# alexmillerdb/two_tower_recommender_model

Hardware: AMD Instinct MI355X
Metric: training pairs/sec at batch 8192 (per GPU) (higher is better)
Workload: dtype fp32; 1 GPU; northstar: 100M items x 50M users, emb_dim 128, towers [128, 64], single-hot uniform ids; global_batch=8192, per_gpu_batch=8192, emb_dim=128, tower_dtype=bf16 (MFMA, fp32 acc), parallelism=single-gpu hipgraph

## Files before the change

### two_tower_recommender_model_amd/csrc/tower.hip

```cpp
#include <vector>

#include "tt_common.h"
#include "dedup.h"
#include "shard.h"

namespace tt {

typedef __attribute__((ext_vector_type(8))) __bf16 bf16x8;
typedef __attribute__((ext_vector_type(4))) float f32x4;
typedef __attribute__((ext_vector_type(4))) __bf16 bf16x4;

constexpr int TR = 32;
constexpr int MAXW = 128;
constexpr int XCH = 128;
constexpr int LSTR = MAXW + 8;
constexpr int FSTR = MAXW + 4;
constexpr int MAXL = 4;

__device__ __forceinline__ int64_t strip_at(int64_t f, int64_t m, int64_t nf) {
  return (((m >> 5) * nf + f) << 5) + (m & 31);
}

struct TowerArgs {
  tt_tower_shape_t s;
// ... 1411 lines not shown
  } else {
#pragma unroll
    for (int mt = 0; mt < MTI; ++mt) {
      const int c = 8 * (mt >> 1) + 2 * q + (mt & 1);
      const f32x4 v = *reinterpret_cast<const f32x4*>(xw + n * IN + 4 * (c ^ n));
      xv[mt] = r >= 0 ? v : (f32x4)(0.f);
    }
#pragma unroll
    for (int s2 = 0; s2 < NI; ++s2) xb[s2] = rk_pack(xv[2 * s2], xv[2 * s2 + 1]);
  }
  uint32_t word = 0u;
  float s_old = 0.f;
  if (UPD) {
    if (blockIdx.x == 0 && threadIdx.x == 0) {
      const int32_t nh = a.dd.ctr[0];
      a.dd.ctr[2] = nh;
      a.dd.ctr[0] = 0;
    }
    word = reinterpret_cast<const uint32_t*>(&a.dd.slots[cl >= 0 ? cl : 0].word)[0];
    s_old = (t ? a.us[1] : a.us[0])[r >= 0 ? r : 0];
  }
  __builtin_amdgcn_sched_barrier(0);
  const char* img0 = wimg + t * RK_IMG_T;
  const char* img1 = img0 + RK_W0 * 256;
  f32x4 acc[8];
  if (!TDBG(512)) rk_strip<NI>(xb, a.xt + (int64_t)t * a.in_max * a.Bp + m * a.in_max, q);
  rk_gemm<8, NI, false>(acc, img0, xb, lane);
  RK_STAMP(4);
  bf16x8 hb[4];
#pragma unroll
  for (int s = 0; s < 4; ++s) {
    f32x4 u0, u1;
#pragma unroll
    for (int j = 0; j < 4; ++j) {
      u0[j] = fmaxf(acc[2 * s][j] + b0v[2 * s][j], 0.f);
      u1[j] = fmaxf(acc[2 * s + 1][j] + b0v[2 * s + 1][j], 0.f);
    }
    hb[s] = rk_pack(u0, u1);
  }
  if (!TDBG(256)) rk_strip<4>(hb, a.act + ((int64_t)t * MAXL + 0) * MAXW * a.Bp + m * MAXW, q);
  f32x4 uo[4];
  rk_gemm<4, 4, false>(acc, img1, hb, lane);
#pragma unroll
  for (int mt = 0; mt < 4; ++mt) uo[mt] = acc[mt];
#pragma unroll
  for (int mt = 0; mt < 4; ++mt) {
#pragma unroll
    for (int j = 0; j < 4; ++j) uo[mt][j] = fmaxf(uo[mt][j] + b1v[mt][j], 0.f);
    const int c = 8 * (mt >> 1) + 2 * q + (mt & 1);
    *reinterpret_cast<f32x4*>(&xo[t][h][n * 64 + ((c ^ n) << 2)]) = uo[mt];
  }
  RK_STAMP(5);
  RK_STAMP(6);
  __syncthreads();
  RK_STAMP(7);
  f32x4 vo[4];
#pragma unroll
  for (int mt = 0; mt < 4; ++mt) {
    const int c = 8 * (mt >> 1) + 2 * q + (mt & 1);
    vo[mt] = *reinterpret_cast<const f32x4*>(&xo[t ^ 1][h][n * 64 + ((c ^ n) << 2)]);
  }
  float gs[4];
#pragma unroll
  for (int mt = 0; mt < 4; ++mt) {
    float e = 0.f;
#pragma unroll
    for (int j = 0; j < 4; ++j) e = fmaf(uo[mt][j], vo[mt][j], e);
    gs[mt] = e;
  }
  float c0 = gs[0] + gs[1], c1 = gs[2] + gs[3];
  c0 += __shfl_xor(c0, 16, 64);
  c1 += __shfl_xor(c1, 16, 64);
  c0 += __shfl_xor(c0, 32, 64);
  c1 += __shfl_xor(c1, 32, 64);
  const float d = c0 + c1;
  float lo = 0.f, dl = 0.f;
  if (live) {
    const float x = d, y = rk_label(lab_raw, a.label_dtype);
    const float e = __expf(-fabsf(x));
    const float l1p = e < 1e-4f ? e * (1.f - 0.5f * e) : __logf(1.f + e);
    const float lsig = fminf(x, 0.f) - l1p;
    lo = (1.f - y) * x - lsig;
    const float rc = __builtin_amdgcn_rcpf(1.f + e);
    dl = ((x >= 0.f ? rc : e * rc) - y) * (a.grad_scale / (float)B);
  }
  if (t == 0 && q == 0) lrow[16 * h + n] = lo;
  float z1[16];
  bf16x8 z1b[4];
#pragma unroll
  for (int mt = 0; mt < 4; ++mt)
#pragma unroll
    for (int j = 0; j < 4; ++j) z1[4 * mt + j] = live && uo[mt][j] > 0.f ? dl * vo[mt][j] : 0.f;
#pragma unroll
  for (int s = 0; s < 2; ++s) {
    bf16x8 v;
#pragma unroll
    for (int j = 0; j < 8; ++j) v[j] = (__bf16)z1[8 * s + j];
    z1b[s] = v;
  }
  RK_STAMP(8);
  rk_gemm<8, 2, true>(acc, img1, z1b, lane);
  float z0[32];
  bf16x8 z0b[4];
#pragma unroll
  for (int mt = 0; mt < 8; ++mt)
#pragma unroll
    for (int j = 0; j < 4; ++j)
      z0[4 * mt + j] = live && (float)hb[mt >> 1][4 * (mt & 1) + j] > 0.f ? acc[mt][j] : 0.f;
#pragma unroll
  for (int s = 0; s < 4; ++s) {
    bf16x8 v;
#pragma unroll
    for (int j = 0; j < 8; ++j) v[j] = (__bf16)z0[8 * s + j];
    z0b[s] = v;
  }
  if (!TDBG(512)) rk_strip<2>(z1b, a.dzt + ((int64_t)t * MAXL + 1) * MAXW * a.Bp + m * MAXW, q);
  if (!TDBG(128)) rk_strip<4>(z0b, a.dzt + ((int64_t)t * MAXL + 0) * MAXW * a.Bp + m * MAXW, q);
  RK_STAMP(9);
  rk_gemm<MTI, 4, true>(acc, img0, z0b, lane);
  RK_STAMP(10);
  float* grow;
  bool store_dx;
  if (IDX) {
    const int32_t po = (int32_t)pout_raw.lo;
    store_dx = r >= 0 && po >= 0;
    grow = (t ? a.gdst[1] : a.gdst[0]) + (int64_t)(store_dx ? po : 0) * IN;
    if (a.xd.W) grow = reinterpret_cast<float*>(px_row(a.xd, store_dx ? po : 0, IN * 4));
  } else {
    grow = live ? a.gpooled + m * a.ldp + a.s.in_col[t] : nullptr;
    store_dx = live;
  }
  if (UPD) {
    float e2[2];
#pragma unroll
    for (int hh = 0; hh < 2; ++hh) {
      const float s0 = rw_sq4(acc[0 + hh]), s1 = rw_sq4(acc[2 + hh]);
      float c2;
      if constexpr (IN == 128) {
        const float s2 = rw_sq4(acc[4 + hh]), s3 = rw_sq4(acc[6 + hh]);
        c2 = (s0 + s2) + (s1 + s3);
      } else {
        c2 = s0 + s1;
      }
      c2 += __shfl_xor(c2, 32, 64);
      c2 += __shfl_xor(c2, 16, 64);
      e2[hh] = c2;
    }
    RK_STAMP2(0);
    const float sq = e2[0] + e2[1];
    const float snew = rw_state(s_old, sq, IN);
    const float step = rw_step(snew, a.ulr, a.ueps);
    const uint32_t cnt = word & (uint32_t)DD_CNT_MASK;
    const bool single = r >= 0 && cl >= 0 && cnt == 1u;
    {
      const bool mul = q == 0 && r >= 0 && cl >= 0 && cnt >= 2u && cnt <= (uint32_t)DD_INL;
      const uint64_t bal = __ballot(mul);
      const int seg = tile * 4 + wid;
      if (seg < a.dd.nseg) {
        if (mul) a.dd.multi[(int64_t)seg * DD_SEGW + 1 + __popcll(bal & ((1ull << lane) - 1))] = cl;
        if (lane == 0) a.dd.multi[(int64_t)seg * DD_SEGW] = __popcll(bal);
      }
    }
#pragma unroll
    for (int mt = 0; mt < MTI; ++mt) {
      const int c = 8 * (mt >> 1) + 2 * q + (mt & 1);
      *reinterpret_cast<f32x4*>(xw + n * IN + 4 * (c ^ n)) = rw_apply(xv[mt], acc[mt], step);
    }
    RK_STAMP2(1);
    asm volatile("" ::: "memory");
    {
      const int rr0 = lane / CPR, pc = lane % CPR;
      float* wtab = t ? a.uw[1] : a.uw[0];
#pragma unroll
      for (int i = 0; i < 16 / RPI; ++i) {
        const int row = RPI * i + rr0;
        const int64_t rid = __shfl((long long)r, row, 64);
        const int sg = __shfl((int)single, row, 64);
        const f32x4 w = *reinterpret_cast<const f32x4*>(xw + row * IN + 4 * pc);
        if (sg) *reinterpret_cast<f32x4*>(wtab + rid * IN + 4 * (pc ^ row)) = w;
      }
    }
    RK_STAMP2(2);
    if (single) {
      if (q == 0) {
        (t ? a.us[1] : a.us[0])[r] = snew;
        a.dd.slots[cl].word = DD_EMPTY;
      }
      store_dx = a.pooled_out != nullptr;
    }
  }
  if (store_dx) {
#pragma unroll
    for (int mt = 0; mt < MTI; ++mt)
      *reinterpret_cast<f32x4*>(grow + 32 * (mt >> 1) + 8 * q + 4 * (mt & 1)) = acc[mt];
  }
  RK_STAMP2(3);
  if (t == 0 && q == 0 && live) a.logits[m] = d;
  if (!IDX && !POOL && a.pooled_out && live) {
    float* prow = a.pooled_out + m * a.ldp + a.s.in_col[t];
#pragma unroll
    for (int mt = 0; mt < MTI; ++mt) *reinterpret_cast<f32x4*>(prow + 32 * (mt >> 1) + 8 * q + 4 * (mt & 1)) = xv[mt];
  }
  RK_STAMP(11);
  RK_STAMP(12);
  rk_colsum<32>(z0, n);
  rk_colsum<16>(z1, n);
  auto feat = [&](int k) { return 32 * ((k >> 2) >> 1) + 8 * q + 4 * ((k >> 2) & 1) + (k & 3); };
  if (h == 1) {
    bsum[t][feat(2 * n)] = z0[0];
    bsum[t][feat(2 * n + 1)] = z0[1];
    bsum[t][RK_W0 + feat(n)] = z1[0];
  }
  RK_STAMP(13);
  __syncthreads();
  RK_STAMP(14);
  if (h == 0) {
    float* db0 = a.dbpart + (((int64_t)t * MAXL + 0) * a.nwg + tile) * MAXW;
    float* db1 = a.dbpart + (((int64_t)t * MAXL + 1) * a.nwg + tile) * MAXW;
    db0[feat(2 * n)] = z0[0] + bsum[t][feat(2 * n)];
    db0[feat(2 * n + 1)] = z0[1] + bsum[t][feat(2 * n + 1)];
    db1[feat(n)] = z1[0] + bsum[t][RK_W0 + feat(n)];
    if (t == 0 && lane == 0) {
      float p = 0.f;
      for (int i = 0; i < TR; ++i) p += lrow[i];
      a.loss_part[tile] = p;
    }
  }
  if (!UPD && a.dd_on && q == 0) dd_insert_defer_finish_at(a.dd, pend, li, tile, 16 * wid + n);
  if constexpr (IDX) {
    if (cpd) *cpd = cpv;
    if (a.xd.W) {
      for (int64_t u = (int64_t)blockIdx.x * cp_per + threadIdx.x + 256; u < cp_end; u += 256) {
        const uint4* s2;
        uint4* d2;
        if (px_copy_unit(a.xd, u, s2, d2)) *d2 = *s2;
      }
    }
    if (a.xd.epoch && blockIdx.x == 0 && threadIdx.x == 0)
      __hip_atomic_fetch_add(a.xd.epoch, 1, __ATOMIC_RELAXED, __HIP_MEMORY_SCOPE_AGENT);
  }
  RK_STAMP(15);
}
template <bool UPD, bool IDX = false, int IN = 128, bool POOL = false>
__global__ void __launch_bounds__(RK_THREADS) tower_rows_kernel(TowerArgs a) {
  tower_rows_body<UPD, IDX, IN, POOL>(a);
}


struct WgradTile {
  int32_t t, l, n0, k0;
};


struct WgradArgs {
  const __bf16* xt;
  const __bf16* act;
  const __bf16* dzt;
  float* slab;
  int64_t P;
  int64_t B;
  int64_t in_max;
  int64_t Bp;
  int S;
  int64_t mslice;
  int ntiles;
  int64_t woff[2][MAXL];
  int64_t boff[2][MAXL];
  int32_t K[2][MAXL];
  int32_t width[MAXL];
  int L;
  const float* dbpart;
  int nwg;
  const float* loss_part;
  float* loss;
  int nbias;
  int64_t tiles_off;
  int64_t* step_state;
  float* adam_pre;
  float lr, beta1, beta2;
  int lds;
  int rm;
  int32_t t2_code[16];
#if TT_EXPERIMENTS
  int64_t* stamps;
#endif
  DedupWs dd;
  int n_res;
};

#if TT_EXPERIMENTS
#define T2_STAMP(k) \
  do { if (a.stamps && threadIdx.x == 0) a.stamps[(int64_t)blockIdx.x * 8 + (k)] = (int64_t)__builtin_amdgcn_s_memrealtime(); } while (0)
#else
#define T2_STAMP(k) do { } while (0)
#endif

constexpr int T2_NT = 64;
constexpr int T2_MB = 32;
constexpr int T2_PF = 8;
constexpr int T2_STR = T2_MB + 8;
constexpr int T2_ROWS = T2_NT + MAXW;
constexpr int T2_LDS = 2 * T2_ROWS * T2_STR * 2;
constexpr int T2_RED = 3 * 64 * 16 * 4;
constexpr int T2_SMEM0 = T2_LDS > T2_RED ? T2_LDS : T2_RED;
constexpr int T2_SMEM = T2_SMEM0 > DD_SMEM ? T2_SMEM0 : DD_SMEM;


__device__ __forceinline__ void wgrad_lds_block(const WgradArgs& a, int lb, char* smem) {
  __bf16* buf = reinterpret_cast<__bf16*>(smem);
  const int tid = threadIdx.x, lane = tid & 63, wid = tid >> 6;
  const int r = lane & 15, q = lane >> 4;
  const int s = __builtin_amdgcn_readfirstlane(lb / a.ntiles), ti = __builtin_amdgcn_readfirstlane(lb % a.ntiles);
  T2_STAMP(0);
  const int code = a.t2_code[ti];
  const int t = code & 15, l = (code >> 4) & 15, n0 = code >> 8;
  const int K = a.K[t][l];
  const int NT = min(T2_NT, a.width[l] - n0);
  const int64_t B = a.B;
  const __bf16* Z = a.dzt + ((int64_t)t * MAXL + l) * MAXW * a.Bp;
  const __bf16* A = l == 0 ? a.xt + (int64_t)t * a.in_max * a.Bp : a.act + ((int64_t)t * MAXL + l - 1) * MAXW * a.Bp;
  const int64_t anf = l == 0 ? a.in_max : MAXW;
  const int64_t mb = (int64_t)s * a.mslice;
  const int64_t me = min(mb + a.mslice, B);
  const int seg = (tid & 3) * 8, frow = tid >> 2;
  const __bf16* src[3];
  int64_t tstr[3];
#pragma unroll
  for (int i = 0; i < 3; ++i) {
    const int f = frow + 64 * i;
    src[i] = f < T2_NT ? (f < NT ? Z + ((int64_t)(n0 + f) << 5) : nullptr)
                       : (f - T2_NT < K ? A + ((int64_t)(f - T2_NT) << 5) : nullptr);
    tstr[i] = (f < T2_NT ? (int64_t)MAXW : anf) << 5;
  }
  const int nh = wid >> 1, kh = wid & 1;
  f32x4 acc[2][4];
#pragma unroll
  for (int i = 0; i < 2; ++i)
#pragma unroll
    for (int j = 0; j < 4; ++j) acc[i][j] = (f32x4)(0.f);
  for (int64_t p0 = mb; p0 < me; p0 += T2_PF * T2_MB) {
    bf16x8 ld[T2_PF][3];
#pragma unroll
    for (int c = 0; c < T2_PF; ++c) {
      const int64_t m = p0 + c * T2_MB + seg;
#pragma unroll
      for (int i = 0; i < 3; ++i)
        ld[c][i] = (src[i] && m < me) ? *reinterpret_cast<const bf16x8*>(src[i] + (m >> 5) * tstr[i] + seg)
                                      : (bf16x8)(__bf16)0.f;
    }
#pragma unroll
    for (int c = 0; c < T2_PF; ++c) {
      if (p0 + c * T2_MB >= me) break;
      __bf16* d = buf + (c & 1) * T2_ROWS * T2_STR;
#pragma unroll
      for (int i = 0; i < 3; ++i)
        if (src[i]) *reinterpret_cast<bf16x8*>(d + (frow + 64 * i) * T2_STR + seg) = ld[c][i];
      __syncthreads();
      if (c == 0 && p0 == mb) T2_STAMP(1);
      bf16x8 fa[2], fb[4];
#pragma unroll
      for (int i = 0; i < 2; ++i) fa[i] = *reinterpret_cast<const bf16x8*>(d + (nh * 32 + i * 16 + r) * T2_STR + q * 8);
#pragma unroll
      for (int j = 0; j < 4; ++j)
        fb[j] = *reinterpret_cast<const bf16x8*>(d + (T2_NT + kh * 64 + j * 16 + r) * T2_STR + q * 8);
#pragma unroll
      for (int i = 0; i < 2; ++i)
#pragma unroll
        for (int j = 0; j < 4; ++j)
          if (nh * 32 + i * 16 < NT && kh * 64 + j * 16 < K)
            acc[i][j] = __builtin_amdgcn_mfma_f32_16x16x32_bf16(fa[i], fb[j], acc[i][j], 0, 0, 0);
    }
  }
  T2_STAMP(2);
  float* dst = a.slab + (int64_t)s * a.P + a.woff[t][l];
#pragma unroll
  for (int i = 0; i < 2; ++i)
#pragma unroll
    for (int j = 0; j < 4; ++j)
      if (nh * 32 + i * 16 < NT && kh * 64 + j * 16 < K)
#pragma unroll
        for (int rr = 0; rr < 4; ++rr) {
          const int n = n0 + nh * 32 + i * 16 + q * 4 + rr;
          const int k = kh * 64 + j * 16 + r;
          dst[(int64_t)n * K + k] = acc[i][j][rr];
        }
  T2_STAMP(3);
}

constexpr int T2R_STR = 208;
static_assert(2 * TR * T2R_STR * 2 <= T2_SMEM, "the row-major staged chunks fit the tail's LDS");
__device__ __forceinline__ bf16x8 t2r_frag(const __bf16* d, int col0, int lane) {
  const int q = lane >> 4, qq = (lane >> 2) & 3, p = lane & 3;
  const __bf16* base = d + (4 * q + qq) * T2R_STR + col0 + 4 * p;
  const bf16x4 lo = __builtin_amdgcn_ds_read_tr16_b64_v4bf16((lds_bf16x4*)base);
  const bf16x4 hi = __builtin_amdgcn_ds_read_tr16_b64_v4bf16((lds_bf16x4*)(base + 16 * T2R_STR));
  return __builtin_shufflevector(lo, hi, 0, 1, 2, 3, 4, 5, 6, 7);
}
__device__ __forceinline__ void wgrad_lds_block_rm(const WgradArgs& a, int lb, char* smem) {
  __bf16* buf = reinterpret_cast<__bf16*>(smem);
  const int tid = threadIdx.x, lane = tid & 63, wid = tid >> 6;
  const int r = lane & 15, q = lane >> 4;
  const int s = __builtin_amdgcn_readfirstlane(lb / a.ntiles), ti = __builtin_amdgcn_readfirstlane(lb % a.ntiles);
  T2_STAMP(0);
  const int code = a.t2_code[ti];
  const int t = code & 15, l = (code >> 4) & 15, n0 = code >> 8;
  const int K = a.K[t][l];
  const int NT = min(T2_NT, a.width[l] - n0);
  const int64_t B = a.B;
  const __bf16* Z = a.dzt + ((int64_t)t * MAXL + l) * MAXW * a.Bp;
  const __bf16* A = l == 0 ? a.xt + (int64_t)t * a.in_max * a.Bp : a.act + ((int64_t)t * MAXL + l - 1) * MAXW * a.Bp;
  const int64_t anf = l == 0 ? a.in_max : MAXW;
  const int64_t mb = (int64_t)s * a.mslice;
  const int64_t me = min(mb + a.mslice, B);
  const char* zb = reinterpret_cast<const char*>(Z);
  const char* ab = reinterpret_cast<const char*>(A);
  const int prow0 = tid >> 3, prow1 = tid >> 4, prow2 = (tid + 256) >> 4;
  const bool ok0 = 8 * (tid & 7) < NT, ok1 = 8 * (tid & 15) < K, ok2 = 8 * ((tid + 256) & 15) < K;
  const uint32_t zstr = MAXW * 2, astr = (uint32_t)anf * 2;
  const uint32_t zo = (uint32_t)(mb + prow0) * zstr + (uint32_t)(n0 + 8 * (tid & 7)) * 2;
  const uint32_t ao1 = (uint32_t)(mb + prow1) * astr + (uint32_t)(8 * (tid & 15)) * 2;
  const uint32_t ao2 = (uint32_t)(mb + prow2) * astr + (uint32_t)(8 * ((tid + 256) & 15)) * 2;
  const int lw0 = prow0 * T2R_STR + 8 * (tid & 7);
  const int lw1 = prow1 * T2R_STR + T2_NT + 8 * (tid & 15);
  const int lw2 = prow2 * T2R_STR + T2_NT + 8 * ((tid + 256) & 15);
  const int nh = wid >> 1, kh = wid & 1;
  f32x4 acc[2][4];
#pragma unroll
  for (int i = 0; i < 2; ++i)
#pragma unroll
    for (int j = 0; j < 4; ++j) acc[i][j] = (f32x4)(0.f);
  for (int64_t p0 = mb; p0 < me; p0 += T2_PF * T2_MB) {
    bf16x8 ld[T2_PF][3];
    const uint32_t dr = (uint32_t)(p0 - mb);
    bool okc[T2_PF][3];
#pragma unroll
    for (int c = 0; c < T2_PF; ++c) {
      const uint32_t rc = dr + c * T2_MB;
      const int64_t mrow = p0 + c * T2_MB;
      okc[c][0] = ok0 && mrow + prow0 < me;
      okc[c][1] = ok1 && mrow + prow1 < me;
      okc[c][2] = ok2 && mrow + prow2 < me;
      ld[c][0] = *reinterpret_cast<const bf16x8*>(zb + zo + (okc[c][0] ? rc * zstr : 0u));
      ld[c][1] = *reinterpret_cast<const bf16x8*>(ab + ao1 + (okc[c][1] ? rc * astr : 0u));
      ld[c][2] = *reinterpret_cast<const bf16x8*>(ab + ao2 + (okc[c][2] ? rc * astr : 0u));
    }
#pragma unroll
    for (int c = 0; c < T2_PF; ++c) {
      if (p0 + c * T2_MB >= me) break;
      __bf16* d = buf + (c & 1) * TR * T2R_STR;
#pragma unroll
      for (int i = 0; i < 3; ++i)
        if (!okc[c][i]) ld[c][i] = (bf16x8)(__bf16)0.f;
      *reinterpret_cast<bf16x8*>(d + lw0) = ld[c][0];
      *reinterpret_cast<bf16x8*>(d + lw1) = ld[c][1];
      *reinterpret_cast<bf16x8*>(d + lw2) = ld[c][2];
      __syncthreads();
      if (c == 0 && p0 == mb) T2_STAMP(1);
      bf16x8 fa[2], fb[4];
#pragma unroll
      for (int i = 0; i < 2; ++i) fa[i] = t2r_frag(d, nh * 32 + i * 16, lane);
#pragma unroll
      for (int j = 0; j < 4; ++j) fb[j] = t2r_frag(d, T2_NT + kh * 64 + j * 16, lane);
#pragma unroll
      for (int i = 0; i < 2; ++i)
#pragma unroll
        for (int j = 0; j < 4; ++j)
          if (nh * 32 + i * 16 < NT && kh * 64 + j * 16 < K)
            acc[i][j] = __builtin_amdgcn_mfma_f32_16x16x32_bf16(fa[i], fb[j], acc[i][j], 0, 0, 0);
    }
  }
  T2_STAMP(2);
  float* dst = a.slab + (int64_t)s * a.P + a.woff[t][l];
#pragma unroll
  for (int i = 0; i < 2; ++i)
#pragma unroll
    for (int j = 0; j < 4; ++j)
      if (nh * 32 + i * 16 < NT && kh * 64 + j * 16 < K)
#pragma unroll
        for (int rr = 0; rr < 4; ++rr) {
          const int n = n0 + nh * 32 + i * 16 + q * 4 + rr;
          const int k = kh * 64 + j * 16 + r;
          dst[(int64_t)n * K + k] = acc[i][j][rr];
        }
  T2_STAMP(3);
}

__device__ __forceinline__ void wgrad_block(const WgradArgs& a, const WgradTile* __restrict__ tiles, int bid,
                                            char* smem) {
  float (*red)[64 * 16] = reinterpret_cast<float (*)[64 * 16]>(smem);
  const int lane = threadIdx.x & 63, wid = threadIdx.x >> 6;
  const int r = lane & 15, q = lane >> 4;
  const int64_t nwg_tiles = (int64_t)a.ntiles * a.S;
  if ((int64_t)bid >= nwg_tiles) {
    T2_STAMP(0);
    int64_t b = ((int64_t)bid - nwg_tiles) * 4 + wid;
    if (b == a.nbias) {
      b = -1;
      if (a.loss) {
        float s = 0.f;
        for (int w0 = 0; w0 < a.nwg; w0 += 512) {
          float v[8];
#pragma unroll
          for (int k = 0; k < 8; ++k) v[k] = w0 + k * 64 + lane < a.nwg ? a.loss_part[w0 + k * 64 + lane] : 0.f;
#pragma unroll
          for (int k = 0; k < 8; ++k) s += v[k];
        }
        s = wave_sum(s);
        if (lane == 0) a.loss[0] = s / (float)a.B;
      }
      if (a.adam_pre && lane == 0) {
        const int64_t t_step = a.step_state[0] + 1;
        a.step_state[0] = t_step;
        const double bc1 = 1.0 - pow((double)a.beta1, (double)t_step);
        const double bc2 = 1.0 - pow((double)a.beta2, (double)t_step);
        a.adam_pre[0] = (float)((double)a.lr / bc1);
        a.adam_pre[1] = (float)sqrt(bc2);
      }
    }
    for (int t = 0; t < 2; ++t)
      for (int l = 0; l < a.L; ++l) {
        if (b >= 0 && b < a.width[l]) {
          const float* dbp = a.dbpart + ((int64_t)t * MAXL + l) * a.nwg * MAXW + b;
          float s = 0.f;
          for (int w0 = 0; w0 < a.nwg; w0 += 512) {
            float v[8];
#pragma unroll
            for (int k = 0; k < 8; ++k) {
              const int w = w0 + k * 64 + lane;
              v[k] = w < a.nwg ? dbp[(int64_t)w * MAXW] : 0.f;
            }
#pragma unroll
            for (int k = 0; k < 8; ++k) s += v[k];
          }
          s = wave_sum(s);
          if (lane == 0) a.slab[a.boff[t][l] + b] = s;
        }
        if (b >= 0) b -= a.width[l];
      }
    T2_STAMP(3);
    return;
  }
  const int lb = xcd_remap(bid, (int)nwg_tiles);
  if (a.lds && a.rm) {
    wgrad_lds_block_rm(a, lb, smem);
    return;
  }
  if (a.lds) {
    wgrad_lds_block(a, lb, smem);
    return;
  }
  const int s = (int)(lb / a.ntiles);
  const WgradTile tl = tiles[lb % a.ntiles];
  const int64_t B = a.B;
  const __bf16* Z = a.dzt + ((int64_t)tl.t * MAXL + tl.l) * MAXW * a.Bp;
  const __bf16* A = tl.l == 0 ? a.xt + (int64_t)tl.t * a.in_max * a.Bp
                              : a.act + ((int64_t)tl.t * MAXL + tl.l - 1) * MAXW * a.Bp;
  const int64_t anf = tl.l == 0 ? a.in_max : MAXW;
  const int64_t mw = a.mslice / 4;
  int64_t mb = (int64_t)s * a.mslice + wid * mw;
  int64_t me = mb + mw;
  if (mb > B) mb = B;
  if (me > B) me = B;
  f32x4 acc[2][2];
  for (int i = 0; i < 2; ++i)
    for (int j = 0; j < 2; ++j) acc[i][j] = (f32x4)(0.f);
  const __bf16* z0 = Z + ((int64_t)(tl.n0 + r) << 5);
  const __bf16* z1 = Z + ((int64_t)(tl.n0 + 16 + r) << 5);
  const __bf16* a0 = A + ((int64_t)(tl.k0 + r) << 5);
  const __bf16* a1 = A + ((int64_t)(tl.k0 + 16 + r) << 5);
  auto zo = [&](int64_t o) { return (((o >> 5) * MAXW) << 5) + (o & 31); };
  auto ao = [&](int64_t o) { return (((o >> 5) * anf) << 5) + (o & 31); };
  int64_t m = mb;
  for (; m + 128 <= me; m += 128) {
    bf16x8 fa0[4], fa1[4], fb0[4], fb1[4];
#pragma unroll
    for (int u = 0; u < 4; ++u) {
      const int64_t o = m + 32 * u + q * 8;
      fa0[u] = *reinterpret_cast<const bf16x8*>(z0 + zo(o));
      fa1[u] = *reinterpret_cast<const bf16x8*>(z1 + zo(o));
      fb0[u] = *reinterpret_cast<const bf16x8*>(a0 + ao(o));
      fb1[u] = *reinterpret_cast<const bf16x8*>(a1 + ao(o));
    }
#pragma unroll
    for (int u = 0; u < 4; ++u) {
      acc[0][0] = __builtin_amdgcn_mfma_f32_16x16x32_bf16(fa0[u], fb0[u], acc[0][0], 0, 0, 0);
      acc[0][1] = __builtin_amdgcn_mfma_f32_16x16x32_bf16(fa0[u], fb1[u], acc[0][1], 0, 0, 0);
      acc[1][0] = __builtin_amdgcn_mfma_f32_16x16x32_bf16(fa1[u], fb0[u], acc[1][0], 0, 0, 0);
      acc[1][1] = __builtin_amdgcn_mfma_f32_16x16x32_bf16(fa1[u], fb1[u], acc[1][1], 0, 0, 0);
    }
  }
  for (; m + 32 <= me; m += 32) {
    const int64_t o = m + q * 8;
    const bf16x8 fa0 = *reinterpret_cast<const bf16x8*>(z0 + zo(o));
    const bf16x8 fa1 = *reinterpret_cast<const bf16x8*>(z1 + zo(o));
    const bf16x8 fb0 = *reinterpret_cast<const bf16x8*>(a0 + ao(o));
    const bf16x8 fb1 = *reinterpret_cast<const bf16x8*>(a1 + ao(o));
    acc[0][0] = __builtin_amdgcn_mfma_f32_16x16x32_bf16(fa0, fb0, acc[0][0], 0, 0, 0);
    acc[0][1] = __builtin_amdgcn_mfma_f32_16x16x32_bf16(fa0, fb1, acc[0][1], 0, 0, 0);
    acc[1][0] = __builtin_amdgcn_mfma_f32_16x16x32_bf16(fa1, fb0, acc[1][0], 0, 0, 0);
    acc[1][1] = __builtin_amdgcn_mfma_f32_16x16x32_bf16(fa1, fb1, acc[1][1], 0, 0, 0);
  }
  if (m < me) {
    bf16x8 fa0, fa1, fb0, fb1;
    for (int j = 0; j < 8; ++j) {
      const int64_t mm = m + q * 8 + j;
      const bool ok = mm < me;
      fa0[j] = ok ? z0[zo(mm)] : (__bf16)0.f;
      fa1[j] = ok ? z1[zo(mm)] : (__bf16)0.f;
      fb0[j] = ok ? a0[ao(mm)] : (__bf16)0.f;
      fb1[j] = ok ? a1[ao(mm)] : (__bf16)0.f;
    }
    acc[0][0] = __builtin_amdgcn_mfma_f32_16x16x32_bf16(fa0, fb0, acc[0][0], 0, 0, 0);
    acc[0][1] = __builtin_amdgcn_mfma_f32_16x16x32_bf16(fa0, fb1, acc[0][1], 0, 0, 0);
    acc[1][0] = __builtin_amdgcn_mfma_f32_16x16x32_bf16(fa1, fb0, acc[1][0], 0, 0, 0);
    acc[1][1] = __builtin_amdgcn_mfma_f32_16x16x32_bf16(fa1, fb1, acc[1][1], 0, 0, 0);
  }
  if (wid > 0) {
#pragma unroll
    for (int i = 0; i < 2; ++i)
#pragma unroll
      for (int j = 0; j < 2; ++j)
#pragma unroll
        for (int rr = 0; rr < 4; ++rr) red[wid - 1][((i * 2 + j) * 4 + rr) * 64 + lane] = acc[i][j][rr];
  }
  __syncthreads();
  if (wid > 0) return;
#pragma unroll
  for (int w = 0; w < 3; ++w)
#pragma unroll
    for (int i = 0; i < 2; ++i)
#pragma unroll
      for (int j = 0; j < 2; ++j)
#pragma unroll
        for (int rr = 0; rr < 4; ++rr) acc[i][j][rr] += red[w][((i * 2 + j) * 4 + rr) * 64 + lane];
  const int K = a.K[tl.t][tl.l];
  float* dst = a.slab + (int64_t)s * a.P + a.woff[tl.t][tl.l];
  for (int i = 0; i < 2; ++i)
    for (int j = 0; j < 2; ++j)
      for (int rr = 0; rr < 4; ++rr) {
        const int n = tl.n0 + i * 16 + q * 4 + rr;
        const int k = tl.k0 + j * 16 + r;
        dst[(int64_t)n * K + k] = acc[i][j][rr];
      }
}

__global__ void __launch_bounds__(256) tower_wgrad_kernel(WgradArgs a, const WgradTile* __restrict__ tiles) {
  __shared__ __attribute__((aligned(16))) char smem[T2_SMEM];
  if ((int)blockIdx.x < a.n_res)
    dd_resolve_block(a.dd, (int)blockIdx.x, a.n_res);
  else
    wgrad_block(a, tiles, (int)blockIdx.x - a.n_res, smem);
}

__global__ void __launch_bounds__(256) tower_wgrad_dedup_kernel(WgradArgs a, const WgradTile* __restrict__ tiles,
                                                                DdUpdateArgs d, int n_t2) {
  __shared__ __attribute__((aligned(16))) char smem[T2_SMEM];
  if ((int)blockIdx.x < n_t2)
    wgrad_block(a, tiles, (int)blockIdx.x, smem);
  else
    dd_update_block(d, (int)blockIdx.x - n_t2, smem);
}

struct InsertArgs {
  const void* col[2];
  int64_t mod[2];
  int32_t tab[2];
  int id_dtype;
  int64_t B;
  DedupWs dd;
  int xcd_wpt;
};
__device__ __forceinline__ int64_t ins_lookup(const InsertArgs& ins, int blk, int tid) {
  if (ins.xcd_wpt <= 0) return (int64_t)blk * 256 + tid;
  const int c = blk & 7, j = blk >> 3;
  const int t = j / ins.xcd_wpt, qi = j - t * ins.xcd_wpt;
  const int64_t b = (int64_t)c * (ins.B / 256) + 8 * qi + (tid >> 5);
  return (int64_t)t * ins.B + 32 * b + (tid & 31);
}

__device__ __forceinline__ void insert_next_block(const InsertArgs& ins, int blk) {
  const int lane = threadIdx.x & 63;
  const int64_t grp = (int64_t)blk * 4 + (threadIdx.x >> 6);
  const int64_t i = grp * 64 + lane;
  DdPend p;
  p.key = DD_EMPTY;
  if (i < 2 * ins.B) {
    const int t = i >= ins.B;
    const int64_t m = i - (t ? ins.B : 0);
    const int64_t id = load_id(t ? ins.col[1] : ins.col[0], ins.id_dtype, m);
    const uint64_t key = id != 0 ? (((uint64_t)(t ? ins.tab[1] : ins.tab[0]) << DD_TABLE_SHIFT) |
                                    (uint64_t)py_mod64(id, t ? ins.mod[1] : ins.mod[0]))
                                 : DD_EMPTY;
    dd_insert_begin(ins.dd, key, (int32_t)i, p);
  }
  if (grp < ins.dd.ovf_groups) dd_insert_defer_finish(ins.dd, p, (int32_t)(i < 2 * ins.B ? i : 0), (int)grp);
}

#if TT_EXPERIMENTS
#define RING_STAMP(p, k) \
  do { if ((p) && threadIdx.x == 0 && blockIdx.x < 2048) (p)[(int64_t)blockIdx.x * 2 + (k)] = (int64_t)__builtin_amdgcn_s_memrealtime(); } while (0)
#else
#define RING_STAMP(p, k) do { (void)(p); } while (0)
#endif

__global__ void __launch_bounds__(256) tower_wgrad_insert_kernel(WgradArgs a, const WgradTile* __restrict__ tiles,
                                                                 InsertArgs ins, int n_t2, int64_t* stamps) {
  __shared__ __attribute__((aligned(16))) char smem[T2_SMEM];
  RING_STAMP(stamps, 0);
  if ((int)blockIdx.x < n_t2)
    wgrad_block(a, tiles, (int)blockIdx.x, smem);
  else
    insert_next_block(ins, (int)blockIdx.x - n_t2);
  RING_STAMP(stamps, 1);
}

__global__ void __launch_bounds__(256, 3) tower_wgrad_route_rowwise_kernel(WgradArgs a, const WgradTile* __restrict__ tiles,
                                                                        RouteArgs r, DdUpdateArgs d, int n_t2,
                                                                        int n_cnt, int n_dd, PxWait w) {
  __shared__ __attribute__((aligned(16))) char smem[T2_SMEM];
  int b = (int)blockIdx.x;
  if (w.W) {
    if (b == 0) px_signal(w);
    if (b == 0 || (n_dd > 0 ? b < n_dd : b >= n_t2 + n_cnt)) px_wait(w);
  }
  if (n_dd > 0) {
    if (b < n_dd) {
      dd_update_block(d, b, smem);
      return;
    }
    b -= n_dd;
    if (b >= n_t2 + n_cnt) return;
  }
  if (b < n_t2) {
    wgrad_block(a, tiles, b, smem);
  } else if (b < n_t2 + n_cnt) {
    const int j = b - n_t2;
    route_count_block(r, j % r.nblk, j / r.nblk, reinterpret_cast<int (*)[RT_MAXW]>(smem));
  } else {
    dd_update_block(d, b - n_t2 - n_cnt, smem);
  }
}

__device__ __forceinline__ void update_block(const UpdateArgs& a, int bid, int nblocks) {
  T3_STAMP(0);
  if (a.wt.W) {
    if (bid == 0) px_signal(a.wt);
    px_wait(a.wt);
  }
// ... 1213 lines not shown
```

Measured before the change: 267.7 million pairs/s.

## Software-pipeline the first wgrad pass with a 3-deep LDS ring and MFMA interleaving

Adds a specialised first pass for full tiles in the row-major weight-gradient kernel. It stages chunks into a 3-slot LDS ring two ahead and prefetches MFMA fragments one chunk ahead. It also uses sched_group_barrier to interleave LDS reads and writes with the MFMAs, and skips MFMAs entirely for waves whose K half is out of range. This is meant to hide LDS latency and cut barriers per chunk, at the cost of more LDS, more registers and extra code paths.

```diff
diff --git a/two_tower_recommender_model_amd/csrc/tower.hip b/two_tower_recommender_model_amd/csrc/tower.hip
--- a/two_tower_recommender_model_amd/csrc/tower.hip
+++ b/two_tower_recommender_model_amd/csrc/tower.hip
@@ -1737,8 +1737,12 @@
 constexpr int T2_ROWS = T2_NT + MAXW;
 constexpr int T2_LDS = 2 * T2_ROWS * T2_STR * 2;
 constexpr int T2_RED = 3 * 64 * 16 * 4;
+constexpr int T2R_STR = 208;
+constexpr int T2R_RING = 3;
+constexpr int T2R_LDS = T2R_RING * TR * T2R_STR * 2;
 constexpr int T2_SMEM0 = T2_LDS > T2_RED ? T2_LDS : T2_RED;
-constexpr int T2_SMEM = T2_SMEM0 > DD_SMEM ? T2_SMEM0 : DD_SMEM;
+constexpr int T2_SMEM1 = T2_SMEM0 > T2R_LDS ? T2_SMEM0 : T2R_LDS;
+constexpr int T2_SMEM = T2_SMEM1 > DD_SMEM ? T2_SMEM1 : DD_SMEM;
 
 
 __device__ __forceinline__ void wgrad_lds_block(const WgradArgs& a, int lb, char* smem) {
@@ -1822,8 +1826,7 @@
   T2_STAMP(3);
 }
 
-constexpr int T2R_STR = 208;
-static_assert(2 * TR * T2R_STR * 2 <= T2_SMEM, "the row-major staged chunks fit the tail's LDS");
+static_assert(T2R_LDS <= T2_SMEM, "the row-major staged chunks fit the tail's LDS");
 __device__ __forceinline__ bf16x8 t2r_frag(const __bf16* d, int col0, int lane) {
   const int q = lane >> 4, qq = (lane >> 2) & 3, p = lane & 3;
   const __bf16* base = d + (4 * q + qq) * T2R_STR + col0 + 4 * p;
@@ -1831,9 +1834,59 @@
   const bf16x4 hi = __builtin_amdgcn_ds_read_tr16_b64_v4bf16((lds_bf16x4*)(base + 16 * T2R_STR));
   return __builtin_shufflevector(lo, hi, 0, 1, 2, 3, 4, 5, 6, 7);
 }
+template <bool ACT>
+__device__ __forceinline__ void t2r_full_pass(const WgradArgs& a, bool more, const bf16x8 (&ld)[T2_PF][3],
+                                              __bf16* buf, int lw0, int lw1, int lw2, int nh, int kh, int lane,
+                                              f32x4 (&acc)[2][4]) {
+  auto stage = [&](int c) {
+    __bf16* d = buf + (c % T2R_RING) * TR * T2R_STR;
+    *reinterpret_cast<bf16x8*>(d + lw0) = ld[c][0];
+    *reinterpret_cast<bf16x8*>(d + lw1) = ld[c][1];
+    *reinterpret_cast<bf16x8*>(d + lw2) = ld[c][2];
+  };
+  auto frags = [&](int c, bf16x8 (&f)[6]) {
+    const __bf16* d = buf + (c % T2R_RING) * TR * T2R_STR;
+#pragma unroll
+    for (int i = 0; i < 2; ++i) f[i] = t2r_frag(d, nh * 32 + i * 16, lane);
+#pragma unroll
+    for (int j = 0; j < 4; ++j) f[2 + j] = t2r_frag(d, T2_NT + kh * 64 + j * 16, lane);
+  };
+  bf16x8 f[2][6];
+  stage(0);
+  stage(1);
+  __syncthreads();
+  T2_STAMP(1);
+  if (ACT) frags(0, f[0]);
+#pragma unroll
+  for (int c = 0; c < T2_PF; ++c) {
+    __builtin_amdgcn_sched_barrier(0);
+    if (c + 2 < T2_PF) stage(c + 2);
+    if (ACT && c + 1 < T2_PF) frags(c + 1, f[(c + 1) & 1]);
+    if (ACT) {
+#pragma unroll
+      for (int j = 0; j < 4; ++j)
+#pragma unroll
+        for (int i = 0; i < 2; ++i)
+          acc[i][j] = __builtin_amdgcn_mfma_f32_16x16x32_bf16(f[c & 1][i], f[c & 1][2 + j],
+                                                              c == 0 ? (f32x4)(0.f) : acc[i][j], 0, 0, 0);
+      if (c + 1 < T2_PF) {
+        if (c + 2 < T2_PF) __builtin_amdgcn_sched_group_barrier(0x200, 3, 0);
+        __builtin_amdgcn_sched_group_barrier(0x8, 1, 0);
+#pragma unroll
+        for (int k = 0; k < 6; ++k) {
+          __builtin_amdgcn_sched_group_barrier(0x8, 1, 0);
+          __builtin_amdgcn_sched_group_barrier(0x100, 2, 0);
+        }
+        __builtin_amdgcn_sched_group_barrier(0x8, 1, 0);
+      }
+    }
+    __builtin_amdgcn_sched_barrier(0);
+    if (c + 2 < T2_PF || (c + 2 == T2_PF && more)) __syncthreads();
+  }
+}
 __device__ __forceinline__ void wgrad_lds_block_rm(const WgradArgs& a, int lb, char* smem) {
   __bf16* buf = reinterpret_cast<__bf16*>(smem);
-  const int tid = threadIdx.x, lane = tid & 63, wid = tid >> 6;
+  const int tid = threadIdx.x, lane = tid & 63, wid = __builtin_amdgcn_readfirstlane(tid >> 6);
   const int r = lane & 15, q = lane >> 4;
   const int s = __builtin_amdgcn_readfirstlane(lb / a.ntiles), ti = __builtin_amdgcn_readfirstlane(lb % a.ntiles);
   T2_STAMP(0);
@@ -1860,11 +1913,41 @@
   const int lw2 = prow2 * T2R_STR + T2_NT + 8 * ((tid + 256) & 15);
   const int nh = wid >> 1, kh = wid & 1;
   f32x4 acc[2][4];
-#pragma unroll
-  for (int i = 0; i < 2; ++i)
-#pragma unroll
-    for (int j = 0; j < 4; ++j) acc[i][j] = (f32x4)(0.f);
-  for (int64_t p0 = mb; p0 < me; p0 += T2_PF * T2_MB) {
+  auto zero_acc = [&]() {
+#pragma unroll
+    for (int i = 0; i < 2; ++i)
+#pragma unroll
+      for (int j = 0; j < 4; ++j) acc[i][j] = (f32x4)(0.f);
+  };
+  const bool full_tile = NT == T2_NT && (K == 64 || K == MAXW);
+  constexpr int64_t PASS = T2_PF * T2_MB;
+  auto full_loads = [&](int64_t p0, bf16x8 (&ld)[T2_PF][3]) {
+    const uint32_t dr = (uint32_t)(p0 - mb);
+#pragma unroll
+    for (int c = 0; c < T2_PF; ++c) {
+      const uint32_t rc = dr + c * T2_MB;
+      ld[c][0] = *reinterpret_cast<const bf16x8*>(zb + zo + rc * zstr);
+      ld[c][1] = *reinterpret_cast<const bf16x8*>(ab + ao1 + (ok1 ? rc * astr : 0u));
+      ld[c][2] = *reinterpret_cast<const bf16x8*>(ab + ao2 + (ok2 ? rc * astr : 0u));
+    }
+  };
+  int64_t p0 = mb;
+  if (full_tile && mb + PASS <= me) {
+    bf16x8 ld[T2_PF][3];
+    full_loads(p0, ld);
+    T2_STAMP(4);
+    const bool more = mb + PASS < me;
+    if (kh * 64 < K) {
+      t2r_full_pass<true>(a, more, ld, buf, lw0, lw1, lw2, nh, kh, lane, acc);
+    } else {
+      zero_acc();
+      t2r_full_pass<false>(a, more, ld, buf, lw0, lw1, lw2, nh, kh, lane, acc);
+    }
+    p0 += PASS;
+  } else {
+    zero_acc();
+  }
+  for (; p0 < me; p0 += PASS) {
     bf16x8 ld[T2_PF][3];
     const uint32_t dr = (uint32_t)(p0 - mb);
     bool okc[T2_PF][3];
@@ -1879,6 +1962,7 @@
       ld[c][1] = *reinterpret_cast<const bf16x8*>(ab + ao1 + (okc[c][1] ? rc * astr : 0u));
       ld[c][2] = *reinterpret_cast<const bf16x8*>(ab + ao2 + (okc[c][2] ? rc * astr : 0u));
     }
+    if (p0 == mb) T2_STAMP(4);
 #pragma unroll
     for (int c = 0; c < T2_PF; ++c) {
       if (p0 + c * T2_MB >= me) break;
```

After: 275.6 million pairs/s (median of 6 runs). +2.9%, better.
